# amazon-science/siam-mot

Hardware: AMD Instinct MI355X
Metric: frame-pairs/sec at 720p, 30 active tracks; EMM xcorr HBM GB/s vs peak (higher is better)
Workload: dtype f32 (towers and correlation: fp16x2 operands on MFMA, fp32 accumulate, fp32-equivalent error); 1 GPU; EMM tracker-head frame pair (EMM.forward + EMM.extract_cache) on DLA-34-FPN 720p FPN maps (net input 704x1280, C=128, 5 levels), 30 tracks, one stream per GPU; hot path only: backbone / RPN / box head / solver are outside the timed region; tracks=30, channels=128, rz=15, rx=30, feature_sets=8, feature_bytes_rotated=307281920

## Files before the change

### siam-mot_amd/csrc/decode.hip

```cpp
#include "smot_common.h"
#include "logit_src.h"
#include "knobs.h"

namespace smot {

__device__ __forceinline__ void cubic_coeffs(float t, float* w) {
    const float A = -0.75f;
    const float x1 = t;
    w[0] = ((A * (x1 + 1.0f) - 5.0f * A) * (x1 + 1.0f) + 8.0f * A) * (x1 + 1.0f) - 4.0f * A;
    w[1] = ((A + 2.0f) * x1 - (A + 3.0f)) * x1 * x1 + 1.0f;
    const float x2 = 1.0f - t;
    w[2] = ((A + 2.0f) * x2 - (A + 3.0f)) * x2 * x2 + 1.0f;
    w[3] = ((A * (x2 + 1.0f) - 5.0f * A) * (x2 + 1.0f) + 8.0f * A) * (x2 + 1.0f) - 4.0f * A;
}

__device__ __forceinline__ void cubic_src(int d, float inv_up, int* base, float* t) {
    const float src = inv_up * ((float)d + 0.5f) - 0.5f;
    const float f = floorf(src);
    *base = (int)f;
    *t = src - f;
}

__device__ __forceinline__ int clampi(int v, int lo, int hi) { return v < lo ? lo : (v > hi ? hi : v); }

// ... 87 lines not shown
constexpr float DEC_TOL = 4e-6f;
constexpr int DEC_REC = 5;
constexpr int DEC_NOM = 64;
constexpr size_t DEC_STATIC_LDS = 6 * 1024;
#if defined(__HIP_DEVICE_COMPILE__) && !defined(__gfx950__) && !defined(__gfx942__) && !defined(__gfx90a__)
#error "decode.hip: the ticket hand-off is written for gfx9 (CDNA) write-through stores"
#endif

typedef __attribute__((address_space(1))) unsigned long long gu64_t;
typedef __attribute__((address_space(1))) unsigned gu32_t;

__device__ __forceinline__ float key_score(unsigned k) {
    if (k == 0xFFFFFFFFu) return __uint_as_float(0x7FC00000u);
    return __uint_as_float((k & 0x80000000u) ? (k & 0x7FFFFFFFu) : ~k);
}

__device__ __forceinline__ unsigned nomination_threshold(unsigned best_key) {
    const float b = key_score(best_key);
    return (fabsf(b) <= 1.0f) ? score_key(b - DEC_TOL) : 0u;
}

struct FinalizeArgs {
    const float* sr;
    float* bb;
    float* conf;
    long long* idx_out;
    unsigned* ticket;
    long long* trace;
    int rx, rz;
    float pad, clip_w, clip_h;
    const int* poison;
};

template <int SPLIT>
__global__ void __launch_bounds__(256 * SPLIT)
decode_kernel(LogitSrc L, const float* __restrict__ boxes, const float* __restrict__ hann, DecodeParams D,
              unsigned long long* __restrict__ cand, FinalizeArgs F) {
    extern __shared__ __attribute__((aligned(16))) float lg[];
    __shared__ unsigned long long wbest[4 * SPLIT];
    __shared__ unsigned nom[DEC_NOM];
    __shared__ int nom_cnt;
    if (threadIdx.x == 0) nom_cnt = 0;
    const int tcol = threadIdx.x & 255, part = threadIdx.x >> 8;
    __shared__ __attribute__((aligned(16))) float wy_tab[32][4];
    __shared__ float hy_tab[32];
    __shared__ float dv[4][4][64];
    const int n = blockIdx.x;
    const int f = (int)blockIdx.y - 1;
    const int Ho = D.Ho, up = D.up, G = D.G;
    const int nband = gridDim.y;
#define DC_TRACE(SLOT)                                                                                          \
    if (F.trace && threadIdx.x == 0)                                                                            \
        F.trace[((size_t)blockIdx.x * gridDim.y + blockIdx.y) * 8 + (SLOT)] = (long long)__builtin_amdgcn_s_memtime();
    DC_TRACE(0)
    if (L.logits != nullptr) {
        for (int e = threadIdx.x; e < 28 * Ho; e += blockDim.x) {
            const int ch = e / (4 * Ho), r = e - ch * 4 * Ho;
            const int k = r / Ho, col = r - k * Ho;
            const int row = clampi(f - 1 + k, 0, Ho - 1);
            lg[ch * Ho * Ho + row * Ho + col] = L.get(n, ch, row * Ho + col, Ho * Ho);
        }
    } else {
        constexpr int NJ = (448 + 256 * SPLIT - 1) / (256 * SPLIT);
        float c2[2];
#pragma unroll
        for (int j = 0; j < NJ; ++j) {
            const int e = threadIdx.x + 256 * SPLIT * j;
            const int ch = e >> 6, row = clampi(f - 1 + ((e >> 4) & 3), 0, Ho - 1);
            c2[j] = (e < 448) ? L.combine(n, ch, row * 16 + (e & 15)) : 0.0f;
        }
#pragma unroll
        for (int j = 0; j < NJ; ++j) {
            const int e = threadIdx.x + 256 * SPLIT * j;
            const int ch = e >> 6, row = clampi(f - 1 + ((e >> 4) & 3), 0, Ho - 1);
            if (e < 448) lg[ch * 256 + row * 16 + (e & 15)] = c2[j];
        }
    }
    const int y_begin = max(0, up * f + up / 2);
    const int y_end = min(G, up * f + up / 2 + up);
    if ((int)threadIdx.x < y_end - y_begin) {
        int by;
        float ty, w4[4];
        cubic_src(y_begin + threadIdx.x, D.inv_up, &by, &ty);
        cubic_coeffs(ty, w4);
        wy_tab[threadIdx.x][0] = w4[0];
        wy_tab[threadIdx.x][1] = w4[1];
        wy_tab[threadIdx.x][2] = w4[2];
        wy_tab[threadIdx.x][3] = w4[3];
        hy_tab[threadIdx.x] = hann[y_begin + threadIdx.x];
    }
    __syncthreads();

    const float box_w = sub_rn(boxes[n * 4 + 2], boxes[n * 4 + 0]);
    const float box_h = sub_rn(boxes[n * 4 + 3], boxes[n * 4 + 1]);
    const float inv_bw = div_rn(1.0f, box_w), inv_bh = div_rn(1.0f, box_h);
    int rows[4];
#pragma unroll
    for (int k = 0; k < 4; ++k) rows[k] = clampi(f - 1 + k, 0, Ho - 1);
    for (int e = threadIdx.x; e < 4 * Ho; e += 256 * SPLIT) {
        const int k = e / Ho, col = e - k * Ho;
        const float* q = lg + rows[k] * Ho + col;
        const int hw = Ho * Ho;
        dv[0][k][col] = (q[0] - q[hw]) * 1.44269504088896341f;
        dv[1][k][col] = q[2 * hw] * -1.44269504088896341f;
        dv[2][k][col] = (q[5 * hw] + q[3 * hw]) * inv_bw;
        dv[3][k][col] = (q[6 * hw] + q[4 * hw]) * inv_bh;
    }
    __syncthreads();
    DC_TRACE(1)
    const int rows_per_part = (y_end - y_begin + SPLIT - 1) / SPLIT;
    const int y0p = y_begin + part * rows_per_part, y1p = min(y_end, y0p + rows_per_part);

    auto walk = [&](int X, int ya, int yb, auto&& visit) {
        int bx;
        float tx, wx[4];
        cubic_src(X, D.inv_up, &bx, &tx);
        cubic_coeffs(tx, wx);
        int cols[4];
#pragma unroll
        for (int k = 0; k < 4; ++k) cols[k] = clampi(bx - 1 + k, 0, Ho - 1);
        float h[4][4];
#pragma unroll
        for (int ch = 0; ch < 4; ++ch)
#pragma unroll
            for (int k = 0; k < 4; ++k) {
                const float* rowp = dv[ch][k];
                h[ch][k] = interp4_fma(rowp[cols[0]], rowp[cols[1]], rowp[cols[2]], rowp[cols[3]], wx);
            }
        const float hx = D.sigma * hann[X];
        for (int Y = ya; Y < yb; ++Y) {
            const float4 w4 = *reinterpret_cast<const float4*>(wy_tab[Y - y_begin]);
            const float wy[4] = {w4.x, w4.y, w4.z, w4.w};
            float v[4];
#pragma unroll
            for (int ch = 0; ch < 4; ++ch) v[ch] = interp4_fma(h[ch][0], h[ch][1], h[ch][2], h[ch][3], wy);
            visit(cell_score_fast(v, hy_tab[Y - y_begin] * hx, D), Y);
        }
    };
    unsigned bsk = 0u, bidx = 0u;
    unsigned sk2 = 0u;
#pragma unroll 1
    for (int j = 0; j < DEC_MAX_COLS; ++j) {
        const int X = tcol + 256 * j;
        if (X >= G) break;
        walk(X, y0p, y1p, [&](float s, int Y) {
            const unsigned sk = score_key(s);
            asm("v_med3_u32 %0, %1, %2, %0" : "+v"(sk2) : "v"(sk), "v"(bsk));
            const bool gt = sk > bsk;
            bsk = gt ? sk : bsk;
            bidx = gt ? (unsigned)(Y * G + X) : bidx;
        });
    }
    const unsigned long long best = bsk != 0u ? (((unsigned long long)bsk << 32) | (unsigned long long)(0xFFFFFFFFu - bidx)) : 0ull;
    DC_TRACE(2)
    const unsigned ws = wave_max_u32((unsigned)(best >> 32));
    const int wave = threadIdx.x >> 6;
    if ((threadIdx.x & 63) == 0) wbest[wave] = ws;
    __syncthreads();
    unsigned wgs = wbest[0];
#pragma unroll
    for (int w = 1; w < 4 * SPLIT; ++w) wgs = max(wgs, wbest[w]);
    const unsigned thr = nomination_threshold(wgs);
// ... 25 lines not shown
    __syncthreads();
    DC_TRACE(4)
    float ev[7];
#pragma unroll
    for (int ch = 0; ch < 7; ++ch) ev[ch] = 0.0f;
    unsigned long long ebest = 0ull;
    {
        const int total = nom_cnt;
        const bool flood = rescore_band || total > DEC_NOM;
        const int cells = flood ? (y_end - y_begin) * G : total;
        const int lane = threadIdx.x & 63;
        const int ch = lane >> 2, k = lane & 3;
        for (int e = wave; e < cells; e += 4 * SPLIT) {
            const unsigned idx = flood ? (unsigned)(y_begin * G + e) : nom[e];
            const int Y = (int)(idx / (unsigned)G), X = (int)(idx - (unsigned)Y * (unsigned)G);
            int bx, by;
            float tx, ty, wx[4], wy[4];
            cubic_src(X, D.inv_up, &bx, &tx);
            cubic_src(Y, D.inv_up, &by, &ty);
            cubic_coeffs(tx, wx);
            cubic_coeffs(ty, wy);
            float hk = 0.0f;
            if (ch < 7) {
                const float* q = lg + ch * Ho * Ho + clampi(by - 1 + k, 0, Ho - 1) * Ho;
                hk = interp4(q[clampi(bx - 1, 0, Ho - 1)], q[clampi(bx, 0, Ho - 1)], q[clampi(bx + 1, 0, Ho - 1)],
                             q[clampi(bx + 2, 0, Ho - 1)], wx);
            }
#define DC_QUAD(K) __int_as_float(__builtin_amdgcn_update_dpp(0, __float_as_int(hk), (K) * 0x55, 0xf, 0xf, false))
            const float vch = interp4(DC_QUAD(0), DC_QUAD(1), DC_QUAD(2), DC_QUAD(3), wy);
#undef DC_QUAD
            float v[7];
#pragma unroll
            for (int c = 0; c < 7; ++c) v[c] = __int_as_float(__builtin_amdgcn_readlane(__float_as_int(vch), 4 * c));
            const float score = cell_score(v, box_w, box_h, mul_rn(hann[Y], hann[X]), D);
            const unsigned long long key = make_key(score, idx);
            if (key > ebest) {
                ebest = key;
#pragma unroll
                for (int c = 0; c < 7; ++c) ev[c] = v[c];
            }
        }
    }
    if ((threadIdx.x & 63) == 0) wbest[wave] = ebest;
    __syncthreads();
    unsigned long long we = wbest[0];
#pragma unroll
    for (int w = 1; w < 4 * SPLIT; ++w) we = (wbest[w] > we) ? wbest[w] : we;

    DC_TRACE(5)
    gu64_t* rec = (gu64_t*)(cand + ((size_t)n * nband + blockIdx.y) * DEC_REC);
    const bool publisher = (we != 0ull) ? (ebest == we) : (wave == 0);
    if (!publisher) return;
    const int lane = threadIdx.x & 63;
    if (lane == 0) {
        if (we == 0ull) {
            __hip_atomic_store(rec, 0ull, __ATOMIC_RELAXED, __HIP_MEMORY_SCOPE_AGENT);
        } else {
            auto pk = [](float a, float b) {
                return ((unsigned long long)__float_as_uint(b) << 32) | (unsigned long long)__float_as_uint(a);
            };
            __hip_atomic_store(rec + 1, pk(ev[0], ev[1]), __ATOMIC_RELAXED, __HIP_MEMORY_SCOPE_AGENT);
            __hip_atomic_store(rec + 2, pk(ev[2], ev[3]), __ATOMIC_RELAXED, __HIP_MEMORY_SCOPE_AGENT);
            __hip_atomic_store(rec + 3, pk(ev[4], ev[5]), __ATOMIC_RELAXED, __HIP_MEMORY_SCOPE_AGENT);
            __hip_atomic_store(rec + 4, pk(ev[6], 0.0f), __ATOMIC_RELAXED, __HIP_MEMORY_SCOPE_AGENT);
            __hip_atomic_store(rec, we, __ATOMIC_RELAXED, __HIP_MEMORY_SCOPE_AGENT);
        }
    }
    asm volatile("s_waitcnt vmcnt(0)" ::: "memory");
    unsigned old = 0u;
    if (lane == 0) old = __hip_atomic_fetch_add((gu32_t*)(F.ticket + n), 1u, __ATOMIC_RELAXED, __HIP_MEMORY_SCOPE_AGENT);
    old = (unsigned)__builtin_amdgcn_readfirstlane((int)old);
    if (F.trace && lane == 0) F.trace[((size_t)blockIdx.x * gridDim.y + blockIdx.y) * 8 + 6] = (long long)__builtin_amdgcn_s_memtime();
    if (old != (unsigned)(nband - 1)) return;

    const float sx1 = F.sr[n * 4 + 0], sy1 = F.sr[n * 4 + 1], sx2 = F.sr[n * 4 + 2], sy2 = F.sr[n * 4 + 3];
    const int poisoned = (F.poison != nullptr) ? *F.poison : 0;
    __builtin_amdgcn_sched_barrier(0);
    const gu64_t* recs = (const gu64_t*)(cand + (size_t)n * nband * DEC_REC);
    unsigned long long bk = 0ull, bw[4] = {0ull, 0ull, 0ull, 0ull};
    for (int b = lane; b < nband; b += 64) {
        const gu64_t* r = recs + (size_t)b * DEC_REC;
        unsigned long long w[DEC_REC];
#pragma unroll
        for (int q = 0; q < DEC_REC; ++q) w[q] = __hip_atomic_load(r + q, __ATOMIC_RELAXED, __HIP_MEMORY_SCOPE_AGENT);
        if (w[0] > bk) {
            bk = w[0];
#pragma unroll
            for (int q = 0; q < 4; ++q) bw[q] = w[1 + q];
        }
    }
    const unsigned long long top = wave_max_u64(bk);
    if (lane == 0) __hip_atomic_store((gu32_t*)(F.ticket + n), 0u, __ATOMIC_RELAXED, __HIP_MEMORY_SCOPE_AGENT);
    if (top == 0ull || bk != top) return;
    float v[8];
#pragma unroll
    for (int q = 0; q < 4; ++q) {
        v[2 * q] = __uint_as_float((unsigned)bw[q]);
        v[2 * q + 1] = __uint_as_float((unsigned)(bw[q] >> 32));
    }
    const unsigned idx = 0xFFFFFFFFu - (unsigned)(top & 0xFFFFFFFFull);
    const int Y = (int)(idx / (unsigned)G), X = (int)(idx - (unsigned)Y * (unsigned)G);
    const int full = F.rx * D.up;
    const int st = (F.rz / 2) * D.up;
    const float stride_w = div_rn(sub_rn(sx2, sx1), (float)(full - 1));
    const float stride_h = div_rn(sub_rn(sy2, sy1), (float)(full - 1));
    const float cx = sub_rn(add_rn(sx1, mul_rn((float)(st + X), stride_w)), F.pad);
    const float cy = sub_rn(add_rn(sy1, mul_rn((float)(st + Y), stride_h)), F.pad);
    float bx1 = sub_rn(cx, v[3]), by1 = sub_rn(cy, v[4]);
    float bx2 = add_rn(cx, v[5]), by2 = add_rn(cy, v[6]);
    if (F.clip_w > 0.0f) {
        bx1 = clamp_nan(bx1, 0.0f, F.clip_w - 1.0f);
        by1 = clamp_nan(by1, 0.0f, F.clip_h - 1.0f);
        bx2 = clamp_nan(bx2, 0.0f, F.clip_w - 1.0f);
        by2 = clamp_nan(by2, 0.0f, F.clip_h - 1.0f);
    }
    const float qnan = __uint_as_float(0x7FC00000u);
    if (poisoned != 0) bx1 = by1 = bx2 = by2 = qnan;
    F.bb[n * 4 + 0] = bx1;
    F.bb[n * 4 + 1] = by1;
    F.bb[n * 4 + 2] = bx2;
    F.bb[n * 4 + 3] = by2;
    const float m = fmaxf(v[0], v[1]);
// ... 17 lines not shown

namespace smot {
unsigned* decode_tickets(float* cand_ws, int N, int Ho) {
    return reinterpret_cast<unsigned*>(cand_ws + (size_t)N * 2 * DEC_REC * (Ho + 1));
}

int decode_impl(LogitSrc L, const float* sr, const float* boxes, const float* hann, int N, int Ho, int up, int rx,
                int rz, float pad_pixels, float one_minus_sigma, float sigma, int use_centerness, float clip_w,
                float clip_h, float* cand_ws, float* bb, float* conf, int64_t* idx, bool tickets_zeroed,
                hipStream_t st, const int* poison) {
    SMOT_REQUIRE(N >= 0 && Ho > 0 && up > 0, "decode: bad sizes N=%d Ho=%d up=%d", N, Ho, up);
    SMOT_REQUIRE(rx - rz + 1 == Ho && (rz & 1) == 1, "decode: need Ho == rx-rz+1 and odd rz (Ho=%d rx=%d rz=%d)", Ho,
                 rx, rz);
    if ((up & (up - 1)) != 0 || up < 2 || up > 32) {
        set_error("decode: up=%d unsupported (power of two in [2,32] required; the reference uses 16)", up);
        return SMOT_ERR_UNSUPPORTED;
    }
    const long long G = (long long)Ho * up;
    SMOT_REQUIRE(G <= 256 * DEC_MAX_COLS, "decode: grid %lld too wide (max %d)", G, 256 * DEC_MAX_COLS);
    const size_t smem = (size_t)7 * Ho * Ho * sizeof(float);
    SMOT_REQUIRE(smem + DEC_STATIC_LDS <= 64 * 1024 && Ho <= 64, "decode: Ho=%d too large for LDS", Ho);
    if (N == 0) return SMOT_OK;
    SMOT_REQUIRE((L.logits || L.part) && sr && boxes && hann && cand_ws && bb && conf, "decode: null pointer");
    SMOT_REQUIRE(((uintptr_t)cand_ws & 7) == 0, "decode: cand_ws must be 8-byte aligned");
    SMOT_REQUIRE(L.logits != nullptr || Ho == 16, "decode: the partial-sum source needs Ho == 16");
    DecodeParams D;
    D.Ho = Ho;
    D.up = up;
    D.G = (int)G;
    D.inv_up = 1.0f / (float)up;
    D.one_minus_sigma = one_minus_sigma;
    D.sigma = sigma;
    D.use_centerness = use_centerness;
    unsigned long long* cand = reinterpret_cast<unsigned long long*>(cand_ws);
    const int split = knobs().decode_split ? knobs().decode_split : (((long long)N * (Ho + 1) <= 768 || G > 256) ? 2 : 1);
#ifdef SMOT_DEBUG
    if (knobs().decode_two_pass) {
        LogitSrc L1 = L;
        if (L.logits == nullptr) SMOT_REQUIRE(L.logits_out != nullptr, "decode (two-pass): needs a logits buffer");
        if (split == 4) {
            hipLaunchKernelGGL(decode_band_kernel<4>, dim3(N, Ho + 1), dim3(1024), smem, st, L1, boxes, hann, D, cand);
        } else if (split == 2) {
            hipLaunchKernelGGL(decode_band_kernel<2>, dim3(N, Ho + 1), dim3(512), smem, st, L1, boxes, hann, D, cand);
        } else {
            hipLaunchKernelGGL(decode_band_kernel<1>, dim3(N, Ho + 1), dim3(256), smem, st, L1, boxes, hann, D, cand);
        }
        int rc2 = check_launch("decode bands");
        if (rc2) return rc2;
        LogitSrc L2 = L;
        if (L.logits == nullptr) L2.logits = L.logits_out;
        hipLaunchKernelGGL(decode_finalize_kernel, dim3(N), dim3(64), 0, st, L2, sr, boxes, hann, D, rx, rz, pad_pixels,
                           (const unsigned long long*)cand, Ho + 1, clip_w, clip_h, bb, conf, (long long*)idx);
        return check_launch("decode finalize");
    }
#endif
    FinalizeArgs F;
    F.sr = sr;
    F.bb = bb;
    F.conf = conf;
    F.idx_out = (long long*)idx;
    F.ticket = decode_tickets(cand_ws, N, Ho);
    F.rx = rx;
    F.rz = rz;
    F.pad = pad_pixels;
    F.clip_w = clip_w;
    F.clip_h = clip_h;
    F.trace = g_trace;
    F.poison = poison;
    if (!tickets_zeroed) {
        hipError_t e = hipMemsetAsync(F.ticket, 0, (size_t)N * sizeof(unsigned), st);
        if (e != hipSuccess) {
            set_error("decode: hipMemsetAsync: %s", hipGetErrorString(e));
            return (int)e;
        }
    }
    if (split == 4) {
        SMOT_LAUNCH(decode_kernel<4>, dim3(N, Ho + 1), dim3(1024), smem, st, L, boxes, hann, D, cand, F);
    } else if (split == 2) {
        SMOT_LAUNCH(decode_kernel<2>, dim3(N, Ho + 1), dim3(512), smem, st, L, boxes, hann, D, cand, F);
    } else {
        SMOT_LAUNCH(decode_kernel<1>, dim3(N, Ho + 1), dim3(256), smem, st, L, boxes, hann, D, cand, F);
    }
    return check_launch("decode");
}
}

extern "C" int smot_emm_decode_fwd(const float* logits, const float* sr, const float* boxes, const float* hann,
                                   int N, int Ho, int up, int rx, int rz, float pad_pixels, float one_minus_sigma,
                                   float sigma, int use_centerness, float clip_w, float clip_h, float* cand_ws,
                                   float* bb, float* conf, int64_t* idx, smot_stream_t stream) {
    smot::LogitSrc L;
    L.logits = logits;
    L.part = nullptr;
    L.tpt = 0;
    L.cls_b = L.center_b = L.reg_b = nullptr;
    L.logits_out = nullptr;
    return smot::decode_impl(L, sr, boxes, hann, N, Ho, up, rx, rz, pad_pixels, one_minus_sigma, sigma,
                             use_centerness, clip_w, clip_h, cand_ws, bb, conf, idx, false, (hipStream_t)stream, nullptr);
}
```

### siam-mot_amd/csrc/logit_src.h

```cpp
#pragma once
#include "smot_common.h"

namespace smot {

struct LogitSrc {
    const float* logits;
    const float* part;
    int tpt;
    const float* cls_b;
    const float* center_b;
    const float* reg_b;
    float* logits_out;

    __device__ __forceinline__ float get(int n, int ch, int pos, int HW) const {
        return logits[((size_t)n * 7 + ch) * HW + pos];
    }

    __device__ __forceinline__ float combine(int n, int ch, int pos) const {
        const int side = ch >= 3;
        const int o = side ? ch - 3 : ch;
        const float* p = part + ((size_t)n * 2 * tpt + side * tpt) * 4 * 256 + (size_t)o * 256 + pos;
        float s = 0.0f;
        for (int t0 = 0; t0 < tpt; t0 += 8) {
            float v[8];
#pragma unroll
            for (int t = 0; t < 8; ++t) v[t] = (t0 + t < tpt) ? p[(size_t)(t0 + t) * 4 * 256] : 0.0f;
#pragma unroll
            for (int t = 0; t < 8; ++t)
                if (t0 + t < tpt) s += v[t];
        }
        s += (ch < 2) ? cls_b[ch] : ((ch == 2) ? center_b[0] : reg_b[ch - 3]);
        return side ? relu_nan(s) : s;
    }
};

}
```

### siam-mot_amd/csrc/tower_wino.hip

```cpp
#include "tower_common.h"
#include "knobs.h"
#include <utility>

namespace smot {

constexpr int W_ROW = 24;
constexpr int W_PLANE = 448;
constexpr int W_STAGE_IC = 8;
constexpr int W_RING = 4;
constexpr int W_BUF = W_STAGE_IC * W_PLANE;
constexpr int W_XOC = 68;
constexpr int W_X_FLOATS = 4 * 2 * 16 * W_XOC;
constexpr int W_PL_OFF = W_X_FLOATS;
constexpr int W_HW_OFF = W_PL_OFF + 16 * T_PLANE;
constexpr int W_ST_OFF = W_HW_OFF + 16 * 36;
constexpr int W_EPI_FLOATS = W_ST_OFF + 32;
constexpr int w_smem_floats(int oct) {
    return (oct * W_EPI_FLOATS > W_RING * W_BUF) ? oct * W_EPI_FLOATS : W_RING * W_BUF;
}
constexpr int W_A_FLOATS = 4 * 4 * 2 * 2 * 256;
constexpr int W_A_SLOT = 4 * 2 * 2 * 256;
constexpr int W_AB_ROW = 4 * 2 * 1024;
static_assert((W_RING * W_BUF + W_A_FLOATS) * 4 <= 160 * 1024, "BF3: ring + A image in one CU's LDS");
static_assert(w_smem_floats(1) * 4 <= 64 * 1024, "OCT = 1: two workgroups per CU, no opt-in needed");
static_assert(w_smem_floats(2) * 4 <= 160 * 1024, "OCT = 2: one workgroup per CU");

__device__ __forceinline__ float tower_pack_scale(unsigned wmax_bits) {
    const int e = (int)((wmax_bits >> 23) & 0xffu);
    if (e == 0 || e == 255) return 1.0f;
    int k = 266 - e;
    k = k < 1 ? 1 : (k > 254 ? 254 : k);
    return __uint_as_float((unsigned)k << 23);
}

__global__ void __launch_bounds__(256)
tower_pack_kernel(const float* __restrict__ wc, const float* __restrict__ wr, int C, float* __restrict__ packed,
                  unsigned* __restrict__ hdr) {
    const int idx = blockIdx.x * 256 + threadIdx.x;
    if (idx >= 2 * C * C) return;
    const int oc = idx / C, ic = idx - oc * C;
    const float* g = (oc < C ? wc + (size_t)oc * C * 9 : wr + (size_t)(oc - C) * C * 9) + (size_t)ic * 9;
    float gg[4][3];
#pragma unroll
    for (int v = 0; v < 3; ++v) {
        const float g0 = g[v], g1 = g[3 + v], g2 = g[6 + v];
        gg[0][v] = g0;
        gg[1][v] = 0.5f * ((g0 + g1) + g2);
        gg[2][v] = 0.5f * ((g0 - g1) + g2);
        gg[3][v] = g2;
    }
    const int tile = oc >> 4, k = ic >> 2, lane = (oc & 15) + 16 * (ic & 3);
    const int nk = C >> 2;
#pragma unroll
    for (int i = 0; i < 4; ++i) {
        float4 u;
        u.x = gg[i][0];
// ... 215 lines not shown
    const int al_wave = __builtin_amdgcn_readfirstlane((xi * 2 + nh) * 512);
    const int al_row = __builtin_amdgcn_readfirstlane(xi * 2 * 512);
    const unsigned long long pa = reinterpret_cast<unsigned long long>(packed);
    const i32x4 rs_a_words = {__builtin_amdgcn_readfirstlane((int)(unsigned)pa),
                              __builtin_amdgcn_readfirstlane((int)((unsigned)(pa >> 32) & 0xffffu)), 0x7fffffff, 0x00020000};
    const unsigned a_lds_byte = (unsigned)(size_t)a_lds;
    auto dma_part = [&](int q, int kbp, int part) __attribute__((always_inline)) {
        const int soff = __builtin_amdgcn_readfirstlane(ab_base + (ABL == 12 ? 0 : kbp) * ab_block + (q * 2 + part) * 1024);
        const unsigned dst = __builtin_amdgcn_readfirstlane(a_lds_byte + (unsigned)(q * W_A_SLOT + al_wave + part * 256) * 4u);
        unsigned keep;
        asm volatile("s_mov_b32 %0, m0\n\ts_mov_b32 m0, %1\n\ts_nop 0\n\tbuffer_load_dwordx4 %2, %3, %4 offen lds\n\ts_mov_b32 m0, %0"
                     : "=&s"(keep) : "s"(dst), "v"(a_voff), "s"(rs_a_words), "s"(soff) : "memory");
    };
    auto dma_slot = [&](int q, int kbp) __attribute__((always_inline)) {
        dma_part(q, kbp, 0);
        dma_part(q, kbp, 1);
    };
    auto load_al = [&](int q, u32x4 (*dst)[2]) __attribute__((always_inline)) {
        const float* src = sm + W_RING * W_BUF + q * W_A_SLOT + al_row + lane * 4;
#pragma unroll
        for (int o = 0; o < OCT; ++o)
#pragma unroll
            for (int part = 0; part < 2; ++part)
                dst[o][part] = *reinterpret_cast<const u32x4*>(src + (o * 2 + part) * 256);
    };
    f32x4 acc[OCT][4][2 * NP];
#pragma unroll
    for (int o = 0; o < OCT; ++o)
#pragma unroll
        for (int q = 0; q < 4; ++q)
#pragma unroll
            for (int t = 0; t < 2 * NP; ++t) acc[o][q][t] = (f32x4){0.f, 0.f, 0.f, 0.f};

    load_raw(0, prs[0]);
    load_raw(1, prs[1]);
    if constexpr (BF3) {
        dma_slot(0, 0);
        dma_slot(1, 0);
    }
    if constexpr (!BF3) load_a(0, aset[0]);
    if (ABL == 2 || ABL >= 5) {
#pragma unroll
        for (int o = 0; o < OCT; ++o) {
            aset[1][0][o] = aset[0][0][o];
            aset[1][1][o] = aset[0][1][o];
        }
    }
    float pmv[2] = {0.0f, 0.0f};
    if constexpr (BF3 && ABL != 10) {
        const float* __restrict__ pmsrc = plane_max + (size_t)n * C;
        if (lane < C) pmv[0] = pmsrc[lane];
        if (lane + 64 < C) pmv[1] = pmsrc[lane + 64];
        __builtin_amdgcn_sched_barrier(0);
    }
    {
        float4* z = reinterpret_cast<float4*>(sm);
        for (int e = tid; e < W_RING * W_BUF / 4; e += NT) z[e] = make_float4(0.f, 0.f, 0.f, 0.f);
    }
    float hwv[9];
    auto load_hwv = [&]() __attribute__((always_inline)) {
        const int o = lane & 3, blk = lane >> 2;
        const float* wsrc = (tower == 1) ? P.reg_w + (size_t)o * C * 9
                                         : (o < 2 ? P.cls_w + (size_t)o * C * 9 : P.center_w);
        const bool live = (tower == 1) || (o < 3);
        wsrc += (size_t)oc0 * 9 + blk;
#pragma unroll
        for (int r = 0; r < 9; ++r) hwv[r] = live ? wsrc[r * 16] : 0.0f;
    };
    if constexpr (!BF3) load_hwv();
    if constexpr (BF3 && ABL != 10) {
        float m = fmaxf(pmv[0], pmv[1]);
        for (int c = lane + 128; c < C; c += 64) m = fmaxf(m, plane_max[(size_t)n * C + c]);
        m = plane_max_wave(m);
        const int e = (int)((__float_as_uint(m) >> 23) & 0xffu);
        if (e != 0 && e != 255) {
            int k = 139 - e;
            k = k < -100 ? -100 : (k > 100 ? 100 : k);
            sv = __uint_as_float((unsigned)(127 + k) << 23);
            inv_sv = __uint_as_float((unsigned)(127 - k) << 23);
        }
    }

    __syncthreads();
    if constexpr (BF3) asm volatile("s_waitcnt vmcnt(0)" ::: "memory");
    store_raw(sm, prs[0]);
    store_raw(sm + W_BUF, prs[1]);
    load_raw(min(2, nstages - 1), prs[0]);
    load_raw(min(3, nstages - 1), prs[1]);
    float ga = 0.0f, be = 0.0f;
    if constexpr (!BLOCKED) {
        ga = P.gamma[tower][oc0 + (ltid >> 4)];
        be = P.beta[tower][oc0 + (ltid >> 4)];
    }
    __syncthreads();

    const int row_a = (xi == 0) ? 0 : ((xi == 2) ? 2 : 1);
    const int row_b = (xi == 2) ? 1 : ((xi == 3) ? 3 : 2);
    const int kq = lane >> 4, xl = lane & 15;
    const int patch0 = kq * W_PLANE + (2 * (xl >> 2) + (OCT == 2 ? 8 * nh : 0)) * W_ROW + 4 * (xl & 3);
    int ia = patch0 + row_a * W_ROW, ib = patch0 + row_b * W_ROW;
    asm volatile("" : "+v"(ia), "+v"(ib));

    float rd[NP][6][2];
    float bop[4][2 * NP];
    if (ABL >= 3) {
#pragma unroll
        for (int e = 0; e < 12 * NP; ++e) {
            (&bop[0][0])[e % (8 * NP)] = (float)(lane + e);
            (&rd[0][0][0])[e] = (float)(lane - e);
        }
    }
#define W_READ(BUFI, Q, RD)                                                                      \
    if (ABL != 3 && (ABL < 5 || ABL >= 7)) {                                                     \
        const float* oa = sm + ia + ((BUFI) * W_BUF + (Q) * 4 * W_PLANE);                        \
        const float* ob = sm + ib + ((BUFI) * W_BUF + (Q) * 4 * W_PLANE);                        \
        _Pragma("unroll") for (int p = 0; p < NP; ++p) {             \
            f32x4 a4 = *reinterpret_cast<const f32x4*>(oa + p * 8 * W_ROW);                      \
            f32x2 a2 = *reinterpret_cast<const f32x2*>(oa + p * 8 * W_ROW + 4);                  \
            f32x4 b4 = *reinterpret_cast<const f32x4*>(ob + p * 8 * W_ROW);                      \
            f32x2 b2 = *reinterpret_cast<const f32x2*>(ob + p * 8 * W_ROW + 4);                  \
            if (BF3) asm volatile("" : "+v"(a4), "+v"(a2), "+v"(b4), "+v"(b2));                  \
            RD[p][0][0] = a4[0]; RD[p][0][1] = b4[0];                                            \
            RD[p][1][0] = a4[1]; RD[p][1][1] = b4[1];                                            \
            RD[p][2][0] = a4[2]; RD[p][2][1] = b4[2];                                            \
            RD[p][3][0] = a4[3]; RD[p][3][1] = b4[3];                                            \
            RD[p][4][0] = a2[0]; RD[p][4][1] = b2[0];                                            \
// ... 157 lines not shown
    }
#define WB_BLOCK(KB) WB_STAGE(0, KB) WB_STAGE(1, KB) WB_STAGE(2, KB) WB_STAGE(3, KB)
#define WB_LOOP                                                                                  \
    W_READ(0, 0, rd)                                                                             \
    W_READ(0, 1, rdb)                                                                            \
    if (nh == 1) asm volatile("s_barrier" ::: "memory");             \
    if (nkb == 4) {                      \
        WB_BLOCK(0) WB_BLOCK(1) WB_BLOCK(2) WB_BLOCK(3)                                          \
    } else if ((nkb & 1) == 0) {                      \
        for (int kb = 0; kb < nkb; kb += 2) { WB_BLOCK(kb) WB_BLOCK(kb + 1) }                    \
    } else {                                                                                     \
        for (int kb = 0; kb < nkb; ++kb) { WB_BLOCK(kb) }                                        \
    }                                                                                            \
                                                                      \
    asm volatile("s_barrier" ::: "memory");                                                      \
    dma_slot(2, nkb);                                                                            \
    asm volatile("s_barrier" ::: "memory");                                                      \
    WB_Q(0)                                                                                      \
    asm volatile("s_waitcnt vmcnt(0)" ::: "memory");                                             \
     \
    _Pragma("unroll") for (int j = 0; j < NRAW; ++j) asm volatile("" :: "v"(prs[0][j].x), "v"(prs[0][j].y), "v"(prs[0][j].z), "v"(prs[0][j].w), \
                                                                    "v"(prs[1][j].x), "v"(prs[1][j].y), "v"(prs[1][j].z), "v"(prs[1][j].w)); \
    asm volatile("s_barrier\n\ts_barrier" ::: "memory");                                         \
    WB_Q(1)                                                                                      \
    asm volatile("s_barrier\n\ts_barrier" ::: "memory");                                         \
    WB_Q(2)                                                                                      \
    if (nh == 0) asm volatile("s_barrier" ::: "memory");
    W_TRACE(1)
    if constexpr (BF3) {
        static_assert(!BF3 || (OCT == 2 && (ABL == 0 || ABL == 7 || ABL == 9 || ABL == 10 || ABL == 12 || ABL == 15)), "BF3: two-tile workgroups only");
        {
            WB_LOOP
        }
        load_hwv();
    } else if (xi == 1) {
        constexpr bool PLUS = true;
        W_LOOP
    } else {
        constexpr bool PLUS = false;
        W_LOOP
    }
    __syncthreads();
#undef WB_LOOP
#undef WB_STAGE
#undef WB_STAMP
#undef WB_BLOCK
#undef WB_XFORM
#undef WB_Q
#undef WB_QM
#undef WB_TERM
#undef WB_MM
#undef WB_SPLIT
#undef WB_CVT
#undef W_LOOP
#undef W_FENCE
#undef W_STAGE
#undef W_MFMA
#undef W_XFORM
#undef W_READ
    W_TRACE(2)

#pragma unroll
    for (int o = 0; o < OCT; ++o)
#pragma unroll
        for (int t = 0; t < 2 * NP; ++t)
#pragma unroll
            for (int r = 0; r < 4; ++r) {
// ... 2 lines not shown
                float* dst = sm + o * W_EPI_FLOATS + ((xi * 2) * 16 + (kq * 4 + r)) * W_XOC +
                             16 * (t + (OCT == 2 ? 2 * nh : 0)) + xl;
                dst[0] = p0;
                dst[16 * W_XOC] = p1;
            }
    float* X = sm + sub * W_EPI_FLOATS;
    float* planes = X + W_PL_OFF;
    float* chs = X + W_ST_OFF;
    for (int e = ltid; e < 16 * 68; e += 256) {
        const int pl = e / 68, c = e - pl * 68;
        const int row = c < 18 ? 0 : (c < 36 ? 17 : 1 + ((c - 36) >> 1));
        const int col = c < 18 ? c : (c < 36 ? c - 18 : (((c - 36) & 1) ? 17 : 0));
        planes[pl * T_PLANE + row * 18 + col] = 0.0f;
    }
    __syncthreads();

    W_TRACE(3)
    const int ocl = ltid >> 4, x16 = ltid & 15;
    float y[4][2][2];
#pragma unroll
    for (int b = 0; b < 2; ++b) {
        const float* src = X + (b * 16 + ocl) * W_XOC + 4 * x16;
        const f32x4 x0 = *reinterpret_cast<const f32x4*>(src + 0 * 32 * W_XOC);
        const f32x4 x1 = *reinterpret_cast<const f32x4*>(src + 1 * 32 * W_XOC);
        const f32x4 x2 = *reinterpret_cast<const f32x4*>(src + 2 * 32 * W_XOC);
        const f32x4 x3 = *reinterpret_cast<const f32x4*>(src + 3 * 32 * W_XOC);
#pragma unroll
        for (int t = 0; t < 4; ++t) {
            y[t][0][b] = (x0[t] + x1[t]) + x2[t];
            y[t][1][b] = (x1[t] - x2[t]) - x3[t];
        }
    }
    if constexpr (BF3) {
        const float inv_su = packed[(size_t)2 * C * C * 16 + (size_t)tiles * (nkb + 1) * 8192 + 1];
#pragma unroll
        for (int t = 0; t < 4; ++t)
#pragma unroll
            for (int a = 0; a < 2; ++a)
#pragma unroll
                for (int b = 0; b < 2; ++b) y[t][a][b] = (y[t][a][b] * inv_sv) * inv_su;
    }

    if constexpr (BLOCKED) {
        constexpr int OV = 32 - BHO;
        float* __restrict__ cdst = part + ((size_t)n * 2 * C + (size_t)tower * C + oc0 + ocl) * MAP;
#pragma unroll
        for (int t = 0; t < 4; ++t) {
            const int ty = (x16 & 3) + 4 * (x16 >> 3), tx = 2 * t + ((x16 >> 2) & 1);
#pragma unroll
            for (int a = 0; a < 2; ++a)
#pragma unroll
                for (int b = 0; b < 2; ++b) {
                    const int lr = 2 * ty + a, lc = 2 * tx + b;
                    if ((oy == 0 || lr >= OV) && (ox == 0 || lc >= OV)) cdst[(oy + lr) * BHO + ox + lc] = y[t][a][b];
                }
        }
        return;
    }
    const float inv_cnt = 1.0f / (float)(cpg * 256);
    float s = 0.0f;
#pragma unroll
    for (int t = 0; t < 4; ++t) s += (y[t][0][0] + y[t][0][1]) + (y[t][1][0] + y[t][1][1]);
    s = group16_sum(s);
    float mean = 0.0f, var = 0.0f;
    const int g0 = (ocl / cpg) * cpg;
    if (cpg == 4) {
#define W_RL(V, L) __int_as_float(__builtin_amdgcn_readlane(__float_as_int(V), (L)))
// ... 63 lines not shown
        __builtin_amdgcn_sched_barrier(0);
        W_HMM(2, 0)
        __builtin_amdgcn_sched_barrier(0);
        W_HMM(3, 1)
#undef W_HMM
#undef W_HLOAD
        hacc[0] += hacc1[0];
        hacc[1] += hacc1[1];
        hacc[2] += hacc1[2];
        hacc[3] += hacc1[3];
        float* __restrict__ dst = part + ((size_t)n * tiles + etile) * 4 * 256 + py * 16 + px;
        dst[0 * 256] = hacc[0];
        dst[1 * 256] = hacc[1];
        dst[2 * 256] = hacc[2];
        dst[3 * 256] = hacc[3];
    }
    W_TRACE(5)
#undef W_TRACE
}

static int tower_tiles_per_workgroup(int N, int C) {
    (void)N;
    (void)C;
    int oct = 2;
    if (knobs().tower_oct == 1 || knobs().tower_oct == 2) oct = knobs().tower_oct;
    return oct;
}

int launch_tower_wino(const float* resp, const float* packed, const TowerParams& P, int N, int C, int cpg, float eps,
                      float* part, unsigned* zero_words, hipStream_t st, const float* plane_max) {
    const int tiles = 2 * (C / 16);
    const int oct = tower_tiles_per_workgroup(N, C);
    const bool bf3 = oct == 2 && knobs().tower_bf3 != 0;
    const size_t smem = (size_t)(bf3 ? W_RING * W_BUF + W_A_FLOATS : w_smem_floats(oct)) * sizeof(float);
    const int grid = ((N + 7) / 8) * 8 * (tiles / oct);
    if (oct == 2) {
        const void* fn = bf3 ? reinterpret_cast<const void*>(&tower_wino_kernel<0, 2, 0, true>)
                             : reinterpret_cast<const void*>(&tower_wino_kernel<0, 2>);
#ifdef SMOT_DEBUG
        if (bf3 && knobs().wino_abl == 7) fn = reinterpret_cast<const void*>(&tower_wino_kernel<7, 2, 0, true>);
        if (bf3 && knobs().wino_abl == 9) fn = reinterpret_cast<const void*>(&tower_wino_kernel<9, 2, 0, true>);
        if (bf3 && knobs().wino_abl == 10) fn = reinterpret_cast<const void*>(&tower_wino_kernel<10, 2, 0, true>);
        if (bf3 && knobs().wino_abl == 12) fn = reinterpret_cast<const void*>(&tower_wino_kernel<12, 2, 0, true>);
        if (bf3 && knobs().wino_abl == 15) fn = reinterpret_cast<const void*>(&tower_wino_kernel<15, 2, 0, true>);
#endif
        const int rco = ensure_lds_optin(fn, smem, "predictor towers (winograd)");
        if (rco) return rco;
    }
    if (bf3) {
        SMOT_REQUIRE(plane_max != nullptr, "predictor towers: the split form needs the response's plane maxima");
#define WB_LAUNCH(A)                                                                                              \
    SMOT_LAUNCH((tower_wino_kernel<A, 2, 0, true>), dim3(grid), dim3(512), smem, st, resp, packed, P, N, C, cpg, eps, part, \
                zero_words, g_trace, plane_max)
#ifdef SMOT_DEBUG
        switch (knobs().wino_abl) {
            case 7: WB_LAUNCH(7); break;
            case 9: WB_LAUNCH(9); break;
            case 10: WB_LAUNCH(10); break;
            case 12: WB_LAUNCH(12); break;
            case 15: WB_LAUNCH(15); break;
            default: WB_LAUNCH(0); break;
        }
#else
        WB_LAUNCH(0);
#endif
#undef WB_LAUNCH
        return check_launch("predictor towers (winograd, fp16 x 2)");
// ... 108 lines not shown
```

Baseline: 18360 frame-pairs/s.

## Hoist global loads early across decode and tower kernels, stage Hann window in LDS

The decode kernel now issues the box, Hann-row and Hann-window loads before the logit staging. When LDS allows, it parks the full Hann window in shared memory and reads it from there in the hot walk and finalize loops. The finalize step loads sr and poison before the ticket atomic, and uses a single fetch when nband <= 64. The tower Winograd kernel hoists the inv_su and head-tap weight loads ahead of the main loop and parks the taps in LDS instead of reloading them from global memory after the loop. The aim is to hide global-load latency; the cost is more LDS per workgroup, which could reduce occupancy, and higher register pressure.

```diff
diff --git a/measure/debug/isa_listing.py b/measure/debug/isa_listing.py
--- /dev/null
+++ b/measure/debug/isa_listing.py
@@ -0,0 +1,85 @@
+import re
+import sys
+
+KEEP = re.compile(r"^\s*(s_load_\w+|s_buffer_load_\w+|global_load_\w+|buffer_load_\w+|flat_load_\w+|global_atomic_\w+|"
+                  r"global_store_\w+|s_waitcnt|s_barrier)\b(.*)$")
+LABEL = re.compile(r"^(\.LBB\d+_\d+):")
+
+
+def kernels(path):
+    name, body = None, []
+    for line in open(path):
+        m = re.match(r"^(_Z\w+):\s", line)
+        if m:
+            name, body = m.group(1), []
+            continue
+        if name is not None:
+            if line.startswith(".Lfunc_end"):
+                yield name, body
+                name = None
+            else:
+                body.append(line.rstrip("\n"))
+
+
+def metadata(path, name):
+    txt = open(path).read()
+    i = txt.find(".name:           %s\n" % name)
+    out = {}
+    if i < 0:
+        return out
+    blk = txt[max(0, txt.rfind("  - .", 0, i) - 4000):i + 2000]
+    for key in (".vgpr_count", ".vgpr_spill_count", ".sgpr_count", ".sgpr_spill_count", ".private_segment_fixed_size",
+                ".group_segment_fixed_size", ".agpr_count"):
+        m = None
+        for m in re.finditer(re.escape(key) + r":\s+(\d+)", blk):
+            pass
+        lo = txt.rfind("\n  - .", 0, i)
+        hi = txt.find("\n  - .", i)
+        own = txt[lo:hi if hi > 0 else len(txt)]
+        m = re.search(re.escape(key) + r":\s+(\d+)", own)
+        if m:
+            out[key] = int(m.group(1))
+    return out
+
+
+def listing(body, full):
+    rows, n_instr = [], 0
+    for line in body:
+        lab = LABEL.match(line)
+        if lab:
+            rows.append(("label", lab.group(1), ""))
+            continue
+        s = line.strip()
+        if not s or s.startswith((";", ".")):
+            continue
+        n_instr += 1
+        m = KEEP.match(line)
+        if m:
+            ops = m.group(2).split(";")[0].strip()
+            rows.append((m.group(1), ops if (full or m.group(1) == "s_waitcnt") else "", n_instr))
+    out, i = [], 0
+    while i < len(rows):
+        op, ops, at = rows[i]
+        if op == "label":
+            if i + 1 < len(rows) and rows[i + 1][0] != "label":
+                out.append("  %s:" % ops)
+            i += 1
+            continue
+        j = i
+        while not full and j + 1 < len(rows) and rows[j + 1][0] == op and rows[j + 1][1] == ops and op != "s_barrier":
+            j += 1
+        cnt = j - i + 1
+        out.append("    [%5d] %s%s %s" % (at, "%d x " % cnt if cnt > 1 else "", op, ops))
+        i = j + 1
+    return out, n_instr
+
+
+if __name__ == "__main__":
+    path, pat = sys.argv[1], sys.argv[2]
+    full = "--full" in sys.argv
+    for name, body in kernels(path):
+        if pat not in name:
+            continue
+        lines, n = listing(body, full)
+        print("%s  (%d instructions)  %s" % (name, n, metadata(path, name)))
+        print("\n".join(lines))
diff --git a/siam-mot_amd/csrc/decode.hip b/siam-mot_amd/csrc/decode.hip
--- a/siam-mot_amd/csrc/decode.hip
+++ b/siam-mot_amd/csrc/decode.hip
@@ -143,7 +143,7 @@
     const int* poison;
 };
 
-template <int SPLIT>
+template <int SPLIT, bool HANN_LDS>
 __global__ void __launch_bounds__(256 * SPLIT)
 decode_kernel(LogitSrc L, const float* __restrict__ boxes, const float* __restrict__ hann, DecodeParams D,
               unsigned long long* __restrict__ cand, FinalizeArgs F) {
@@ -155,6 +155,7 @@
     const int tcol = threadIdx.x & 255, part = threadIdx.x >> 8;
     __shared__ __attribute__((aligned(16))) float wy_tab[32][4];
     __shared__ float hy_tab[32];
+    float* const hann_s = lg + 7 * D.Ho * D.Ho;
     __shared__ float dv[4][4][64];
     const int n = blockIdx.x;
     const int f = (int)blockIdx.y - 1;
@@ -164,6 +165,21 @@
     if (F.trace && threadIdx.x == 0)                                                                            \
         F.trace[((size_t)blockIdx.x * gridDim.y + blockIdx.y) * 8 + (SLOT)] = (long long)__builtin_amdgcn_s_memtime();
     DC_TRACE(0)
+    unsigned boff = (unsigned)n * 4u;
+    asm volatile("" : "+v"(boff));
+    const float tb0 = boxes[boff + 0], tb1 = boxes[boff + 1], tb2 = boxes[boff + 2], tb3 = boxes[boff + 3];
+    const int y_begin = max(0, up * f + up / 2);
+    const int y_end = min(G, up * f + up / 2 + up);
+    const bool row_lane = (int)threadIdx.x < y_end - y_begin;
+    const float hyv = row_lane ? hann[y_begin + threadIdx.x] : 0.0f;
+    constexpr int NHS = DEC_MAX_COLS / SPLIT;
+    float hsv[NHS];
+#pragma unroll
+    for (int j = 0; j < NHS; ++j) {
+        const int i = threadIdx.x + 256 * SPLIT * j;
+        hsv[j] = (HANN_LDS && i < G) ? hann[i] : 0.0f;
+    }
+    __builtin_amdgcn_sched_barrier(0);
     if (L.logits != nullptr) {
         for (int e = threadIdx.x; e < 28 * Ho; e += blockDim.x) {
             const int ch = e / (4 * Ho), r = e - ch * 4 * Ho;
@@ -187,9 +203,18 @@
             if (e < 448) lg[ch * 256 + row * 16 + (e & 15)] = c2[j];
         }
     }
-    const int y_begin = max(0, up * f + up / 2);
-    const int y_end = min(G, up * f + up / 2 + up);
-    if ((int)threadIdx.x < y_end - y_begin) {
+    if constexpr (HANN_LDS) {
+#pragma unroll
+        for (int j = 0; j < NHS; ++j) {
+            const int i = threadIdx.x + 256 * SPLIT * j;
+            if (i < G) hann_s[i] = hsv[j];
+        }
+    }
+    auto window = [&](int i) {
+        if constexpr (HANN_LDS) return hann_s[i];
+        else return hann[i];
+    };
+    if (row_lane) {
         int by;
         float ty, w4[4];
         cubic_src(y_begin + threadIdx.x, D.inv_up, &by, &ty);
@@ -198,12 +223,12 @@
         wy_tab[threadIdx.x][1] = w4[1];
         wy_tab[threadIdx.x][2] = w4[2];
         wy_tab[threadIdx.x][3] = w4[3];
-        hy_tab[threadIdx.x] = hann[y_begin + threadIdx.x];
+        hy_tab[threadIdx.x] = hyv;
     }
     __syncthreads();
 
-    const float box_w = sub_rn(boxes[n * 4 + 2], boxes[n * 4 + 0]);
-    const float box_h = sub_rn(boxes[n * 4 + 3], boxes[n * 4 + 1]);
+    const float box_w = sub_rn(tb2, tb0);
+    const float box_h = sub_rn(tb3, tb1);
     const float inv_bw = div_rn(1.0f, box_w), inv_bh = div_rn(1.0f, box_h);
     int rows[4];
 #pragma unroll
@@ -238,7 +263,7 @@
                 const float* rowp = dv[ch][k];
                 h[ch][k] = interp4_fma(rowp[cols[0]], rowp[cols[1]], rowp[cols[2]], rowp[cols[3]], wx);
             }
-        const float hx = D.sigma * hann[X];
+        const float hx = D.sigma * window(X);
         for (int Y = ya; Y < yb; ++Y) {
             const float4 w4 = *reinterpret_cast<const float4*>(wy_tab[Y - y_begin]);
             const float wy[4] = {w4.x, w4.y, w4.z, w4.w};
@@ -330,7 +355,7 @@
             float v[7];
 #pragma unroll
             for (int c = 0; c < 7; ++c) v[c] = __int_as_float(__builtin_amdgcn_readlane(__float_as_int(vch), 4 * c));
-            const float score = cell_score(v, box_w, box_h, mul_rn(hann[Y], hann[X]), D);
+            const float score = cell_score(v, box_w, box_h, mul_rn(hy_tab[Y - y_begin], window(X)), D);
             const unsigned long long key = make_key(score, idx);
             if (key > ebest) {
                 ebest = key;
@@ -364,6 +389,8 @@
             __hip_atomic_store(rec, we, __ATOMIC_RELAXED, __HIP_MEMORY_SCOPE_AGENT);
         }
     }
+    const float sx1 = F.sr[n * 4 + 0], sy1 = F.sr[n * 4 + 1], sx2 = F.sr[n * 4 + 2], sy2 = F.sr[n * 4 + 3];
+    const int poisoned = (F.poison != nullptr) ? *F.poison : 0;
     asm volatile("s_waitcnt vmcnt(0)" ::: "memory");
     unsigned old = 0u;
     if (lane == 0) old = __hip_atomic_fetch_add((gu32_t*)(F.ticket + n), 1u, __ATOMIC_RELAXED, __HIP_MEMORY_SCOPE_AGENT);
@@ -371,12 +398,9 @@
     if (F.trace && lane == 0) F.trace[((size_t)blockIdx.x * gridDim.y + blockIdx.y) * 8 + 6] = (long long)__builtin_amdgcn_s_memtime();
     if (old != (unsigned)(nband - 1)) return;
 
-    const float sx1 = F.sr[n * 4 + 0], sy1 = F.sr[n * 4 + 1], sx2 = F.sr[n * 4 + 2], sy2 = F.sr[n * 4 + 3];
-    const int poisoned = (F.poison != nullptr) ? *F.poison : 0;
-    __builtin_amdgcn_sched_barrier(0);
     const gu64_t* recs = (const gu64_t*)(cand + (size_t)n * nband * DEC_REC);
     unsigned long long bk = 0ull, bw[4] = {0ull, 0ull, 0ull, 0ull};
-    for (int b = lane; b < nband; b += 64) {
+    auto fetch = [&](int b) {
         const gu64_t* r = recs + (size_t)b * DEC_REC;
         unsigned long long w[DEC_REC];
 #pragma unroll
@@ -386,6 +410,11 @@
 #pragma unroll
             for (int q = 0; q < 4; ++q) bw[q] = w[1 + q];
         }
+    };
+    if (nband <= 64) {
+        if (lane < nband) fetch(lane);
+    } else {
+        for (int b = lane; b < nband; b += 64) fetch(b);
     }
     const unsigned long long top = wave_max_u64(bk);
     if (lane == 0) __hip_atomic_store((gu32_t*)(F.ticket + n), 0u, __ATOMIC_RELAXED, __HIP_MEMORY_SCOPE_AGENT);
@@ -469,6 +498,8 @@
     D.one_minus_sigma = one_minus_sigma;
     D.sigma = sigma;
     D.use_centerness = use_centerness;
+    const bool hann_lds = smem + (size_t)G * sizeof(float) + DEC_STATIC_LDS <= 64 * 1024;
+    const size_t smem_launch = smem + (hann_lds ? (size_t)G * sizeof(float) : 0);
     unsigned long long* cand = reinterpret_cast<unsigned long long*>(cand_ws);
     const int split = knobs().decode_split ? knobs().decode_split : (((long long)N * (Ho + 1) <= 768 || G > 256) ? 2 : 1);
 #ifdef SMOT_DEBUG
@@ -511,13 +542,20 @@
             return (int)e;
         }
     }
+#define DEC_LAUNCH(S)                                                                                                  \
+    if (hann_lds) {                                                                                                    \
+        SMOT_LAUNCH((decode_kernel<S, true>), dim3(N, Ho + 1), dim3(256 * S), smem_launch, st, L, boxes, hann, D, cand, F); \
+    } else {                                                                                                           \
+        SMOT_LAUNCH((decode_kernel<S, false>), dim3(N, Ho + 1), dim3(256 * S), smem_launch, st, L, boxes, hann, D, cand, F); \
+    }
     if (split == 4) {
-        SMOT_LAUNCH(decode_kernel<4>, dim3(N, Ho + 1), dim3(1024), smem, st, L, boxes, hann, D, cand, F);
+        DEC_LAUNCH(4)
     } else if (split == 2) {
-        SMOT_LAUNCH(decode_kernel<2>, dim3(N, Ho + 1), dim3(512), smem, st, L, boxes, hann, D, cand, F);
+        DEC_LAUNCH(2)
     } else {
-        SMOT_LAUNCH(decode_kernel<1>, dim3(N, Ho + 1), dim3(256), smem, st, L, boxes, hann, D, cand, F);
-    }
+        DEC_LAUNCH(1)
+    }
+#undef DEC_LAUNCH
     return check_launch("decode");
 }
 }
diff --git a/siam-mot_amd/csrc/logit_src.h b/siam-mot_amd/csrc/logit_src.h
--- a/siam-mot_amd/csrc/logit_src.h
+++ b/siam-mot_amd/csrc/logit_src.h
@@ -20,6 +20,7 @@
         const int side = ch >= 3;
         const int o = side ? ch - 3 : ch;
         const float* p = part + ((size_t)n * 2 * tpt + side * tpt) * 4 * 256 + (size_t)o * 256 + pos;
+        const float bias = (ch < 2) ? cls_b[ch] : ((ch == 2) ? center_b[0] : reg_b[ch - 3]);
         float s = 0.0f;
         for (int t0 = 0; t0 < tpt; t0 += 8) {
             float v[8];
@@ -29,7 +30,7 @@
             for (int t = 0; t < 8; ++t)
                 if (t0 + t < tpt) s += v[t];
         }
-        s += (ch < 2) ? cls_b[ch] : ((ch == 2) ? center_b[0] : reg_b[ch - 3]);
+        s += bias;
         return side ? relu_nan(s) : s;
     }
 };
diff --git a/siam-mot_amd/csrc/tower_wino.hip b/siam-mot_amd/csrc/tower_wino.hip
--- a/siam-mot_amd/csrc/tower_wino.hip
+++ b/siam-mot_amd/csrc/tower_wino.hip
@@ -21,7 +21,9 @@
 constexpr int W_A_FLOATS = 4 * 4 * 2 * 2 * 256;
 constexpr int W_A_SLOT = 4 * 2 * 2 * 256;
 constexpr int W_AB_ROW = 4 * 2 * 1024;
-static_assert((W_RING * W_BUF + W_A_FLOATS) * 4 <= 160 * 1024, "BF3: ring + A image in one CU's LDS");
+constexpr int W_HWP_OFF = W_RING * W_BUF + W_A_FLOATS;
+constexpr int W_HWP_FLOATS = 9 * 512;
+static_assert((W_HWP_OFF + W_HWP_FLOATS) * 4 <= 160 * 1024, "BF3: ring + A image + parked head taps in one CU's LDS");
 static_assert(w_smem_floats(1) * 4 <= 64 * 1024, "OCT = 1: two workgroups per CU, no opt-in needed");
 static_assert(w_smem_floats(2) * 4 <= 160 * 1024, "OCT = 2: one workgroup per CU");
 
@@ -303,31 +305,6 @@
 #pragma unroll
             for (int t = 0; t < 2 * NP; ++t) acc[o][q][t] = (f32x4){0.f, 0.f, 0.f, 0.f};
 
-    load_raw(0, prs[0]);
-    load_raw(1, prs[1]);
-    if constexpr (BF3) {
-        dma_slot(0, 0);
-        dma_slot(1, 0);
-    }
-    if constexpr (!BF3) load_a(0, aset[0]);
-    if (ABL == 2 || ABL >= 5) {
-#pragma unroll
-        for (int o = 0; o < OCT; ++o) {
-            aset[1][0][o] = aset[0][0][o];
-            aset[1][1][o] = aset[0][1][o];
-        }
-    }
-    float pmv[2] = {0.0f, 0.0f};
-    if constexpr (BF3 && ABL != 10) {
-        const float* __restrict__ pmsrc = plane_max + (size_t)n * C;
-        if (lane < C) pmv[0] = pmsrc[lane];
-        if (lane + 64 < C) pmv[1] = pmsrc[lane + 64];
-        __builtin_amdgcn_sched_barrier(0);
-    }
-    {
-        float4* z = reinterpret_cast<float4*>(sm);
-        for (int e = tid; e < W_RING * W_BUF / 4; e += NT) z[e] = make_float4(0.f, 0.f, 0.f, 0.f);
-    }
     float hwv[9];
     auto load_hwv = [&]() __attribute__((always_inline)) {
         const int o = lane & 3, blk = lane >> 2;
@@ -336,8 +313,39 @@
         const bool live = (tower == 1) || (o < 3);
         wsrc += (size_t)oc0 * 9 + blk;
 #pragma unroll
-        for (int r = 0; r < 9; ++r) hwv[r] = live ? wsrc[r * 16] : 0.0f;
+        for (int r = 0; r < 9; ++r) {
+            const float w = wsrc[r * 16];
+            hwv[r] = live ? w : 0.0f;
+        }
     };
+    load_raw(0, prs[0]);
+    load_raw(1, prs[1]);
+    if constexpr (BF3) {
+        dma_slot(0, 0);
+        dma_slot(1, 0);
+    }
+    float inv_su = 1.0f;
+    if constexpr (BF3) inv_su = packed[(size_t)2 * C * C * 16 + (size_t)tiles * ((C >> 5) + 1) * 8192 + 1];
+    if constexpr (!BF3) load_a(0, aset[0]);
+    if (ABL == 2 || ABL >= 5) {
+#pragma unroll
+        for (int o = 0; o < OCT; ++o) {
+            aset[1][0][o] = aset[0][0][o];
+            aset[1][1][o] = aset[0][1][o];
+        }
+    }
+    float pmv[2] = {0.0f, 0.0f};
+    if constexpr (BF3 && ABL != 10) {
+        const float* __restrict__ pmsrc = plane_max + (size_t)n * C;
+        if (lane < C) pmv[0] = pmsrc[lane];
+        if (lane + 64 < C) pmv[1] = pmsrc[lane + 64];
+        __builtin_amdgcn_sched_barrier(0);
+    }
+    if constexpr (BF3 && !BLOCKED) load_hwv();
+    {
+        float4* z = reinterpret_cast<float4*>(sm);
+        for (int e = tid; e < W_RING * W_BUF / 4; e += NT) z[e] = make_float4(0.f, 0.f, 0.f, 0.f);
+    }
     if constexpr (!BF3) load_hwv();
     if constexpr (BF3 && ABL != 10) {
         float m = fmaxf(pmv[0], pmv[1]);
@@ -363,6 +371,11 @@
         ga = P.gamma[tower][oc0 + (ltid >> 4)];
         be = P.beta[tower][oc0 + (ltid >> 4)];
     }
+    if constexpr (BF3 && !BLOCKED) {
+#pragma unroll
+        for (int r = 0; r < 9; ++r) sm[W_HWP_OFF + r * NT + tid] = hwv[r];
+    }
+    if constexpr (BF3) asm volatile("" :: "s"(inv_su));
     __syncthreads();
 
     const int row_a = (xi == 0) ? 0 : ((xi == 2) ? 2 : 1);
@@ -586,7 +599,10 @@
         {
             WB_LOOP
         }
-        load_hwv();
+        if constexpr (!BLOCKED) {
+#pragma unroll
+            for (int r = 0; r < 9; ++r) hwv[r] = sm[W_HWP_OFF + r * NT + tid];
+        }
     } else if (xi == 1) {
         constexpr bool PLUS = true;
         W_LOOP
@@ -655,7 +671,6 @@
         }
     }
     if constexpr (BF3) {
-        const float inv_su = packed[(size_t)2 * C * C * 16 + (size_t)tiles * (nkb + 1) * 8192 + 1];
 #pragma unroll
         for (int t = 0; t < 4; ++t)
 #pragma unroll
@@ -785,7 +800,7 @@
     const int tiles = 2 * (C / 16);
     const int oct = tower_tiles_per_workgroup(N, C);
     const bool bf3 = oct == 2 && knobs().tower_bf3 != 0;
-    const size_t smem = (size_t)(bf3 ? W_RING * W_BUF + W_A_FLOATS : w_smem_floats(oct)) * sizeof(float);
+    const size_t smem = (size_t)(bf3 ? W_HWP_OFF + W_HWP_FLOATS : w_smem_floats(oct)) * sizeof(float);
     const int grid = ((N + 7) / 8) * 8 * (tiles / oct);
     if (oct == 2) {
         const void* fn = bf3 ? reinterpret_cast<const void*>(&tower_wino_kernel<0, 2, 0, true>)
```

Result: no change. 18270 frame-pairs/s (-0.5%).
